# YuliangXiu/ICON

Hardware: NVIDIA H100
Metric: M query-points/sec at 256^3 grid (higher is better)
Workload: dtype f32

## Files before the change

icon_b200/csrc/common.cuh:

```cuda
#pragma once
#include <cuda_runtime.h>
#include <stdint.h>
#include <stdio.h>

#include "../../include/icon_b200.h"

namespace icon {

void set_error(const char *fmt, ...);
void count_launch(int n = 1);

#define ICON_CHECK_ARG(cond, ...)                 \
    do {                                          \
        if (!(cond)) {                            \
            icon::set_error(__VA_ARGS__);         \
            return ICON_EINVAL;                   \
        }                                         \
    } while (0)

#define ICON_CUDA(expr)                                                              \
    do {                                                                             \
        cudaError_t _e = (expr);                                                     \
        if (_e != cudaSuccess) {                                                     \
            icon::set_error("%s:%d %s -> %s", __FILE__, __LINE__, #expr,             \
// ... 57 lines not shown
    template <typename T>
    T *take(size_t n) {
        off = align_up(off, 256);
        T *r = (T *)(base ? base + off : nullptr);
        off += n * sizeof(T);
        return r;
    }
    size_t total() const { return align_up(off, 256); }
};

constexpr int BVH_MAX_LEVELS = 10;
constexpr int RAY_GRID = 256;
constexpr int RAY_LIST_PER_FACE = 64;

constexpr int BRICK_AX = 32;
constexpr int NBRICK = BRICK_AX * BRICK_AX * BRICK_AX;
constexpr int BRICK_MAX_LEAVES = 4096;
constexpr int64_t BRICK_LIST_CAP = 1 << 24;
static inline int64_t brick_list_cap(int F) {
    const int64_t all = (int64_t)NBRICK * ((F + 3) / 4);
    return all < BRICK_LIST_CAP ? all : BRICK_LIST_CAP;
}

struct MeshHeader {
    float y0, z0, inv_cy, inv_cz;
    int ray_overflow;
    int brick_built;
    int brick_overflow;
    int pad;
};

struct MeshView {
    const float4 *tri;
    const float4 *sph;
    const float4 *attr;
    const float4 *rbox;
    float *vnormals;
    unsigned long long *keys;
    int32_t *order;
    float4 *tri_s;
    float4 *sph_s;
    float4 *nodes;
    int32_t *rcount;
    int32_t *roff;
    int32_t *rlist;
    MeshHeader *hdr;
    void *scan_ws;
    float4 *bxyz;
    int32_t *bperm;
    float *brec;
    int32_t *bface;
    float *bub;
    int32_t *boff;
    unsigned short *blist;
    int64_t brick_cap;
    int V, F;
    int nlevels;
    int lvl_cnt[BVH_MAX_LEVELS];
    int lvl_off[BVH_MAX_LEVELS];
};
size_t mesh_ws_bytes(int V, int F);
MeshView mesh_view(const void *ws, int V, int F);
void bricks_forget(const MeshView &m);

void profile_mark(int i, cudaStream_t stream);

size_t scan_ws_bytes(int64_t n);
int scan_exclusive_i32(const int32_t *in, int32_t *out, int64_t n, int64_t *d_total ,
                       void *ws, cudaStream_t stream);

}
```

icon_b200/csrc/mlp.cu:

```cuda
#include "common.cuh"
#include "query_common.cuh"

namespace icon {

constexpr int MP = 64;
constexpr int MT = 256;
constexpr int KC = 16;

constexpr int OFF_W0 = 0;
constexpr int OFF_B0 = OFF_W0 + 16 * 512;
constexpr int OFF_W1 = OFF_B0 + 512;
constexpr int OFF_B1 = OFF_W1 + 512 * 256;
constexpr int OFF_W2 = OFF_B1 + 256;
constexpr int OFF_B2 = OFF_W2 + 272 * 128;
constexpr int OFF_W3 = OFF_B2 + 128;
constexpr int OFF_B3 = OFF_W3 + 144;
static_assert(OFF_B3 + 1 == ICON_MLP_PACKED_FLOATS, "packed layout");

template <int MODE>
__global__ void __launch_bounds__(MT, 2) k_query_mlp(QueryParams q) {
    extern __shared__ __align__(16) float sm[];
    float *x0s = sm;
    float *stage = sm + 16 * MP;
    float *h1s = stage + 10240;
// ... 168 lines not shown
        const float *hb = (st < 16 ? h1s + (size_t)st * KC * MP : x0s) + tx * 4;
#pragma unroll
        for (int k = 0; k < KC; ++k) {
            float4 a0 = *(const float4 *)(wb + k * 128);
            float4 b0 = *(const float4 *)(hb + k * MP), b1 = *(const float4 *)(hb + k * MP + 32);
            float a[4] = {a0.x, a0.y, a0.z, a0.w};
            float b[8] = {b0.x, b0.y, b0.z, b0.w, b1.x, b1.y, b1.z, b1.w};
#pragma unroll
            for (int i = 0; i < 4; ++i)
#pragma unroll
                for (int j = 0; j < 8; ++j) acc2[i][j] = fmaf(a[i], b[j], acc2[i][j]);
        }
        __syncthreads();
    }

    float part[8];
#pragma unroll
    for (int j = 0; j < 8; ++j) part[j] = 0.f;
#pragma unroll
    for (int i = 0; i < 4; ++i) {
        const int ch = ty * 4 + i;
        const float bia = __ldg(W + OFF_B2 + ch), w3 = __ldg(W + OFF_W3 + ch);
#pragma unroll
        for (int j = 0; j < 8; ++j) part[j] = fmaf(w3, lrelu(acc2[i][j] + bia), part[j]);
    }
#pragma unroll
    for (int j = 0; j < 8; ++j) {
        part[j] += __shfl_xor_sync(0xffffffffu, part[j], 8);
        part[j] += __shfl_xor_sync(0xffffffffu, part[j], 16);
    }
    const int lane = tid & 31, wid = tid >> 5;
    if (lane < 8) {
#pragma unroll
        for (int j = 0; j < 4; ++j) {
            red[wid * MP + lane * 4 + j] = part[j];
            red[wid * MP + 32 + lane * 4 + j] = part[4 + j];
        }
    }
    __syncthreads();
    if (tid < MP) {
        const int64_t pi = p0 + tid;
        if (pi < q.N) {
            float s = 0.f;
#pragma unroll
            for (int w = 0; w < 8; ++w) s += red[w * MP + tid];
            for (int j = 0; j < 16; ++j) s = fmaf(__ldg(W + OFF_W3 + 128 + j), x0s[j * MP + tid], s);
            s += __ldg(W + OFF_B3);
            float in_cube = (MODE == 3) ? 1.f : q.xyz4[pi].w;
            q.out[pi] = in_cube * s;
        }
    }
}

__global__ void k_outlier_flag(const float *__restrict__ rec, int64_t N, float clip, int32_t *__restrict__ flag) {
    int64_t i = (int64_t)blockIdx.x * blockDim.x + threadIdx.x;
    if (i < N) flag[i] = fabsf(rec[8 * i]) >= clip ? 1 : 0;
}
__global__ void k_outlier_signs(const float *__restrict__ rec, int64_t N, float clip,
                                const int32_t *__restrict__ krank, int8_t *__restrict__ signs) {
    int64_t i = (int64_t)blockIdx.x * blockDim.x + threadIdx.x;
    if (i < N) {
        float s = rec[8 * i];
        if (fabsf(s) >= clip) signs[krank[i]] = s > 0.f ? 1 : -1;
    }
}

constexpr size_t MLP_SMEM = (16 * MP + 10240 + 256 * MP) * sizeof(float);

template <int MODE>
static int launch_mlp(const QueryParams &q, cudaStream_t stream) {
    static bool attr_set[ICON_MAX_DEVICES] = {};
    if (device_needs_setup(attr_set))
        ICON_CUDA(cudaFuncSetAttribute(k_query_mlp<MODE>, cudaFuncAttributeMaxDynamicSharedMemorySize, (int)MLP_SMEM));
    unsigned nblk = (unsigned)((q.N + MP - 1) / MP);
    k_query_mlp<MODE><<<nblk, MT, MLP_SMEM, stream>>>(q);
    ICON_LAUNCHED();
    return ICON_OK;
}

int launch_mlp_tc(int mode, const QueryParams &q, const void *blob, cudaStream_t stream);
static int g_mlp_impl = 1;

template <int MODE>
static int launch_any(const QueryParams &q, const void *tc, cudaStream_t stream) {
    if (g_mlp_impl == 1) {
        if (!tc) {
            set_error("icon_query / icon_mlp_only: the tensor-core MLP needs the packed tensor-core weight blob (mlp_tc == NULL); "
                      "pass it or select the FP32 kernel with icon_set_mlp_impl(0)");
            return ICON_EINVAL;
        }
        if (q.c0 > 15) {
            set_error("icon_query / icon_mlp_only: the tensor-core MLP takes c0 <= 15 input channels (got %d)", q.c0);
            return ICON_EINVAL;
        }
        return launch_mlp_tc(MODE, q, tc, stream);
    }
    return launch_mlp<MODE>(q, stream);
}

size_t sdf_ws_bytes(int64_t N);
int run_sdf(const float *points, int64_t sc, int64_t sn, int64_t N, const float *h_calib, const MeshView &m,
            float *rec, int32_t *face, void *ws, float4 **xyz4_out, cudaStream_t stream);
int run_points_only(const float *points, int64_t sc, int64_t sn, int64_t N, const float *h_calib,
                    float4 *xyz4, cudaStream_t stream);

struct QueryWs {
    void *sdf_ws;
    float *rec;
    int32_t *krank;
    int8_t *signs;
    int64_t *d_K;
    void *scan_ws;
    float4 *xyz4;
};

static QueryWs carve_query(Carver &c, int64_t N, int prior) {
    QueryWs w{};
    if (prior == ICON_PRIOR_ICON) {
        w.sdf_ws = c.take<char>(sdf_ws_bytes(N));
        w.rec = c.take<float>((size_t)N * 8);
        w.krank = c.take<int32_t>((size_t)N);
        w.signs = c.take<int8_t>((size_t)N);
        w.d_K = c.take<int64_t>(1);
        w.scan_ws = c.take<char>(scan_ws_bytes(N));
    } else {
        w.xyz4 = c.take<float4>((size_t)N);
    }
    return w;
}

}

using namespace icon;

extern "C" size_t icon_query_workspace_bytes(int64_t N, int F, int prior) {
    (void)F;
    Carver c(nullptr);
    carve_query(c, N, prior);
    return c.total();
}

extern "C" int icon_query(int prior, const float *points, int64_t stride_c, int64_t stride_n, int64_t N,
                          const float *h_calib, const float *feat, int C, int H, int W,
                          const float *vol_feat, int VD, const void *mesh_ws, int V, int F,
                          const float *mlp_packed, const void *mlp_tc, int c0, float sdf_clip, float *out,
                          void *ws, size_t ws_bytes, icon_stream_t stream_) {
    cudaStream_t stream = (cudaStream_t)stream_;
    ICON_CHECK_ARG(N >= 0 && N < (int64_t)INT32_MAX, "icon_query: N=%lld out of range", (long long)N);
    if (N == 0) return ICON_OK;
    ICON_CHECK_ARG(points && h_calib && feat && mlp_packed && out && ws, "icon_query: null pointer");
    ICON_CHECK_ARG(((uintptr_t)mlp_tc & 15) == 0, "icon_query: mlp_tc must be 16-byte aligned");
    ICON_CHECK_ARG(c0 >= 1 && c0 <= 16, "icon_query: c0=%d unsupported (1..16)", c0);
    ICON_CHECK_ARG(H >= 2 && W >= 2, "icon_query: feature map %dx%d too small", H, W);
    {
        Carver c(nullptr);
        carve_query(c, N, prior);
        if (ws_bytes < c.total()) {
            set_error("icon_query: workspace %zu < %zu", ws_bytes, c.total());
            return ICON_ENOSPC;
        }
    }
    Carver c(ws);
    QueryWs w = carve_query(c, N, prior);
    QueryParams q{};
    q.feat = feat; q.C = C; q.H = H; q.W = W; q.vol = vol_feat; q.VD = VD;
    q.mlp = mlp_packed; q.c0 = c0; q.clip = sdf_clip; q.out = out; q.N = N;
    if (prior == ICON_PRIOR_ICON) {
        ICON_CHECK_ARG(mesh_ws && V > 0 && F > 0, "icon_query: icon prior needs a prepared body mesh");
        ICON_CHECK_ARG(C % 2 == 0 && C / 2 + 7 == c0, "icon_query: icon prior expects c0 = C/2 + 7 (C=%d c0=%d)", C, c0);
        MeshView m = mesh_view(mesh_ws, V, F);
        float4 *xyz4 = nullptr;
        int rc = run_sdf(points, stride_c, stride_n, N, h_calib, m, w.rec, nullptr, w.sdf_ws, &xyz4, stream);
        if (rc) return rc;
        unsigned nb = (unsigned)((N + 255) / 256);
        k_outlier_flag<<<nb, 256, 0, stream>>>(w.rec, N, sdf_clip, w.krank);
        ICON_LAUNCHED();
        rc = scan_exclusive_i32(w.krank, w.krank, N, w.d_K, w.scan_ws, stream);
        if (rc) return rc;
        k_outlier_signs<<<nb, 256, 0, stream>>>(w.rec, N, sdf_clip, w.krank, w.signs);
        ICON_LAUNCHED();
        q.xyz4 = xyz4; q.rec = w.rec; q.krank = w.krank; q.signs = w.signs; q.d_K = w.d_K;
        profile_mark(3, stream);
        rc = launch_any<0>(q, mlp_tc, stream);
        profile_mark(4, stream);
        return rc;
    }
    profile_mark(0, stream);
    int rc = run_points_only(points, stride_c, stride_n, N, h_calib, w.xyz4, stream);
    if (rc) return rc;
    profile_mark(1, stream); profile_mark(2, stream); profile_mark(3, stream);
    q.xyz4 = w.xyz4;
    if (prior == ICON_PRIOR_PIFU) {
        ICON_CHECK_ARG(C + 1 == c0, "icon_query: pifu prior expects c0 = C + 1 (C=%d c0=%d)", C, c0);
        rc = launch_any<1>(q, mlp_tc, stream);
        profile_mark(4, stream);
        return rc;
    }
    if (prior == ICON_PRIOR_PAMIR) {
        ICON_CHECK_ARG(vol_feat && VD >= 2 && C + 7 == c0, "icon_query: pamir prior expects vol_feat and c0 = C + 7");
        rc = launch_any<2>(q, mlp_tc, stream);
        profile_mark(4, stream);
        return rc;
    }
    set_error("icon_query: unknown prior %d", prior);
    return ICON_EINVAL;
}

extern "C" int icon_set_mlp_impl(int impl) {
    ICON_CHECK_ARG(impl == 0 || impl == 1, "icon_set_mlp_impl: 0 (fp32) or 1 (tensor cores)");
    g_mlp_impl = impl;
    return ICON_OK;
}
extern "C" int icon_get_mlp_impl(void) { return g_mlp_impl; }

extern "C" int icon_mlp_only(const float *feature, int c0, int64_t N, const float *mlp_packed, const void *mlp_tc,
                             float *out, icon_stream_t stream_) {
    cudaStream_t stream = (cudaStream_t)stream_;
    if (N == 0) return ICON_OK;
    ICON_CHECK_ARG(feature && mlp_packed && out && c0 >= 1 && c0 <= 16, "icon_mlp_only: bad argument");
    QueryParams q{};
    q.raw = feature; q.mlp = mlp_packed; q.c0 = c0; q.out = out; q.N = N;
    return launch_any<3>(q, mlp_tc, stream);
}
```

icon_b200/csrc/sdf.cu:

```cuda
#include <float.h>
#include <stdlib.h>

#include <algorithm>
#include <mutex>
#include <type_traits>
#include <unordered_set>

#include "common.cuh"
#include "geom.cuh"

namespace icon {

struct Calib {
    float r[9];
    float t[3];
};

__device__ __forceinline__ V3 load_point(const float *__restrict__ pts, int64_t sc, int64_t sn,
                                         int64_t i, const Calib &cb) {
    float px = pts[i * sn], py = pts[sc + i * sn], pz = pts[2 * sc + i * sn];
    V3 o;
    o.x = fmaf(cb.r[2], pz, fmaf(cb.r[1], py, cb.r[0] * px)) + cb.t[0];
    o.y = fmaf(cb.r[5], pz, fmaf(cb.r[4], py, cb.r[3] * px)) + cb.t[1];
    o.z = fmaf(cb.r[8], pz, fmaf(cb.r[7], py, cb.r[6] * px)) + cb.t[2];
    return o;
}

__device__ __forceinline__ void emit_record(V3 p, int bi, float best, int hits, const MeshView &m,
                                            float *__restrict__ rec, int32_t *__restrict__ face,
                                            int64_t idx) {
    Tri t = load_tri(m.tri + 3 * (size_t)bi);
    V3 n = cross3(t.ab, t.ac);
    float s = n.x * n.x + n.y * n.y + n.z * n.z;
    if (s == 0.f) s = 1e-6f;
    float inv = 1.0f / s;
    V3 w = sub3(p, t.a);
    V3 uw = cross3(t.ab, w), wv = cross3(w, t.ac);
    float b2 = (uw.x * n.x + uw.y * n.y + uw.z * n.z) * inv;
    float b1 = (wv.x * n.x + wv.y * n.y + wv.z * n.z) * inv;
    float b0 = 1.0f - b1 - b2;
    const float4 *at = m.attr + 6 * (size_t)bi;
    float4 a0 = __ldg(at), a1 = __ldg(at + 1), a2 = __ldg(at + 2), a3 = __ldg(at + 3),
           a4 = __ldg(at + 4), a5 = __ldg(at + 5);
    float nx = (a0.x * b0 + a0.w * b1 + a1.z * b2) * -1.f;
    float ny = (a0.y * b0 + a1.x * b1 + a1.w * b2) * 1.f;
    float nz = (a0.z * b0 + a1.y * b1 + a2.x * b2) * -1.f;
    float cx = a2.y * b0 + a3.x * b1 + a3.w * b2;
    float cy = a2.z * b0 + a3.y * b1 + a4.x * b2;
    float cz = a2.w * b0 + a3.z * b1 + a4.y * b2;
    float vv = a4.z * b0 + a4.w * b1 + a5.x * b2;
    float vis = vv >= 0.1f ? 1.f : 0.f;
    float dist = sqrtf(best) / sqrtf(3.0f);
    float sign = 2.0f * ((float)(hits & 1) - 0.5f);
    float sdf = dist * sign;
    float4 *r = (float4 *)(rec + 8 * idx);
    r[0] = make_float4(sdf, cx, cy, cz);
    r[1] = make_float4(nx, ny, nz, vis);
    if (face) face[idx] = bi;
}

constexpr int SW_T = 128;
constexpr int NBIN_AX = 128;
constexpr int NBIN = NBIN_AX * NBIN_AX * NBIN_AX;
__host__ __device__ constexpr int fr_cap(int ppw) { return ppw >= 16 ? 1024 : (ppw >= 4 ? 768 : 384); }

__device__ __forceinline__ float box_dist2(V3 p, float4 lo, float4 hi) {
    float dx = fmaxf(fmaxf(lo.x - p.x, p.x - hi.x), 0.f);
    float dy = fmaxf(fmaxf(lo.y - p.y, p.y - hi.y), 0.f);
    float dz = fmaxf(fmaxf(lo.z - p.z, p.z - hi.z), 0.f);
    return fmaf(dz, dz, fmaf(dy, dy, dx * dx));
}

__device__ __forceinline__ unsigned spread7(unsigned v) {
    v = (v | (v << 16)) & 0x030000FFu;
    v = (v | (v << 8)) & 0x0300F00Fu;
    v = (v | (v << 4)) & 0x030C30C3u;
    v = (v | (v << 2)) & 0x09249249u;
    return v;
}

__device__ __forceinline__ int bin_of(V3 p) {
    const bool inside = p.x >= -1.f && p.x <= 1.f && p.y >= -1.f && p.y <= 1.f && p.z >= -1.f && p.z <= 1.f;
    if (!inside) return NBIN;
    const unsigned bx = min(NBIN_AX - 1, (int)((p.x + 1.f) * (NBIN_AX * 0.5f)));
    const unsigned by = min(NBIN_AX - 1, (int)((p.y + 1.f) * (NBIN_AX * 0.5f)));
    const unsigned bz = min(NBIN_AX - 1, (int)((p.z + 1.f) * (NBIN_AX * 0.5f)));
    return (int)(spread7(bx) | (spread7(by) << 1) | (spread7(bz) << 2));
}

__global__ void k_points_bin(const float *__restrict__ pts, int64_t sc, int64_t sn, int64_t N, Calib cb,
                             float4 *__restrict__ xyz4, int32_t *__restrict__ bid, int32_t *__restrict__ count) {
    const int64_t i = (int64_t)blockIdx.x * blockDim.x + threadIdx.x;
    const bool live = i < N;
    int b = -1;
    if (live) {
        const V3 p = load_point(pts, sc, sn, i, cb);
        const float in_cube = (p.x > -1.f && p.x < 1.f && p.y > -1.f && p.y < 1.f && p.z > -1.f && p.z < 1.f) ? 1.f : 0.f;
        xyz4[i] = make_float4(p.x, p.y, p.z, in_cube);
        b = bin_of(p);
        bid[i] = b;
    }
    const unsigned act = __ballot_sync(0xffffffffu, live);
    if (live) {
        const unsigned peers = __match_any_sync(act, b);
        if ((int)(threadIdx.x & 31) == __ffs(peers) - 1) atomicAdd(&count[b], __popc(peers));
    }
}

__global__ void k_points_scatter(const int32_t *__restrict__ bid, int64_t N, const int32_t *__restrict__ offset,
                                 int32_t *__restrict__ cursor, int32_t *__restrict__ perm) {
    const int64_t i = (int64_t)blockIdx.x * blockDim.x + threadIdx.x;
// ... 17 lines not shown
__device__ __forceinline__ float warp_min(float v) {
    for (int o = 16; o; o >>= 1) v = fminf(v, __shfl_xor_sync(0xffffffffu, v, o));
    return v;
}

#ifdef ICON_SDF_STATS
__device__ unsigned long long g_stats[8];
#define STAT(i, v) do { if (lane == 0) atomicAdd(&g_stats[i], (unsigned long long)(v)); } while (0)
#else
#define STAT(i, v) do { } while (0)
#endif

struct ChunkSmem {
    float4 sph[32];
    float4 tri[32][3];
    int kk[32];
};
template <int FR_CAP>
struct WarpSmem : ChunkSmem {
    unsigned short fr[2][FR_CAP];
};
template <int PPW, bool BRICK>
using SdfSmem = typename std::conditional<BRICK, ChunkSmem, WarpSmem<fr_cap(PPW)>>::type;
template <int PPW, bool BRICK>
constexpr size_t sdf_smem_bytes() { return sizeof(SdfSmem<PPW, BRICK>) * (SW_T / 32); }

constexpr float BRICK_W = 2.0f / BRICK_AX;
constexpr float BRICK_HALF_DIAG = 0.0541266f;

__device__ __forceinline__ void brick_box(int b, float4 &lo, float4 &hi) {
    const int bx = b % BRICK_AX, by = (b / BRICK_AX) % BRICK_AX, bz = b / (BRICK_AX * BRICK_AX);
    lo = make_float4(-1.f + bx * BRICK_W, -1.f + by * BRICK_W, -1.f + bz * BRICK_W, 0.f);
    hi = make_float4(-1.f + (bx + 1) * BRICK_W, -1.f + (by + 1) * BRICK_W, -1.f + (bz + 1) * BRICK_W, 0.f);
}

__device__ __forceinline__ float leaf_key(const MeshView &m, int l, float4 lo, float4 hi) {
    const float4 a = __ldg(m.nodes + 2 * (size_t)l), z = __ldg(m.nodes + 2 * (size_t)l + 1);
    const float gx = fmaxf(fmaxf(a.x - hi.x, lo.x - z.x), 0.f);
    const float gy = fmaxf(fmaxf(a.y - hi.y, lo.y - z.y), 0.f);
    const float gz = fmaxf(fmaxf(a.z - hi.z, lo.z - z.z), 0.f);
    return fmaf(gz, gz, fmaf(gy, gy, gx * gx));
}

__device__ __forceinline__ float box_far2(V3 p, float4 lo, float4 hi) {
    float dx = fmaxf(fabsf(lo.x - p.x), fabsf(hi.x - p.x));
    float dy = fmaxf(fabsf(lo.y - p.y), fabsf(hi.y - p.y));
    float dz = fmaxf(fabsf(lo.z - p.z), fabsf(hi.z - p.z));
    return fmaf(dz, dz, fmaf(dy, dy, dx * dx));
}

template <int PPW, bool BRICK>
__device__ __forceinline__ void sdf_warp(int64_t wid, SdfSmem<PPW, BRICK> &S, const float4 *__restrict__ xyz4,
                                         const int32_t *__restrict__ perm, int64_t N, const MeshView &m,
                                         float *__restrict__ rec, int32_t *__restrict__ face, int order,
                                         int32_t *__restrict__ defer, int32_t *__restrict__ ndefer) {
    constexpr int REP = 32 / PPW;
    constexpr int FR_CAP = fr_cap(PPW);
    const int lane = threadIdx.x & 31;
    const int sub = lane % PPW, rep_id = lane / PPW;
    const int64_t pos0 = wid * PPW;
    const int64_t pos = pos0 + sub;
    if (pos0 >= N) return;
    const bool live = pos < N;
    const int64_t idx = perm[live ? pos : pos0];
    const float4 q = xyz4[idx];
    const V3 p = mk3(q.x, q.y, q.z);
    const V3 c = mk3(0.5f * (warp_min(p.x) + warp_max(p.x)), 0.5f * (warp_min(p.y) + warp_max(p.y)),
                     0.5f * (warp_min(p.z) + warp_max(p.z)));
    const float rw = warp_max(sqrtf(dot3(sub3(p, c), sub3(p, c)))) * 1.00001f + 1e-6f;
    const float4 wlo = make_float4(warp_min(p.x) - 1e-6f, warp_min(p.y) - 1e-6f, warp_min(p.z) - 1e-6f, 0.f);
    const float4 whi = make_float4(warp_max(p.x) + 1e-6f, warp_max(p.y) + 1e-6f, warp_max(p.z) + 1e-6f, 0.f);
    const MeshHeader h = *m.hdr;

    float best = FLT_MAX;
    int bi = 0x7fffffff;
    float ubw2;
    int cur = 0, n = 1;
    bool overflow = false;
    int b = 0;
    float4 blo, bhi;
    if constexpr (BRICK) {
        bool ok = h.brick_built && !h.brick_overflow && c.x >= -1.f && c.x < 1.f && c.y >= -1.f && c.y < 1.f &&
                  c.z >= -1.f && c.z < 1.f;
        if (ok) {
            const int bx = min(BRICK_AX - 1, (int)((c.x + 1.f) * (BRICK_AX * 0.5f)));
            const int by = min(BRICK_AX - 1, (int)((c.y + 1.f) * (BRICK_AX * 0.5f)));
            const int bz = min(BRICK_AX - 1, (int)((c.z + 1.f) * (BRICK_AX * 0.5f)));
            b = (bz * BRICK_AX + by) * BRICK_AX + bx;
            brick_box(b, blo, bhi);
            ok = wlo.x >= blo.x && wlo.y >= blo.y && wlo.z >= blo.z && whi.x <= bhi.x && whi.y <= bhi.y && whi.z <= bhi.z;
        }
        if (!ok) {
            if (lane == 0) defer[atomicAdd(ndefer, 1)] = (int32_t)wid;
            return;
        }
        const int f = __ldg(m.bface + b);
        const Tri tr = load_tri(m.tri + 3 * (size_t)f);
        best = tri_sqdist(p, tr.a, tr.ab, tr.ac);
        bi = f;
        ubw2 = fminf(warp_max(sqrtf(best)), __ldg(m.bub + b));
        STAT(0, 1);
    } else {
        auto try_face = [&](int k) {
            const Tri tr = load_tri(m.tri_s + 3 * (size_t)k);
            const float d = tri_sqdist(p, tr.a, tr.ab, tr.ac);
            const int f = __ldg(m.order + k);
            if (d < best || (d == best && f < bi)) { best = d; bi = f; }
// ... 58 lines not shown
        }
        if (order && !overflow && n > 8) {
            const float ubmin = warp_min(best * rsqrtf(fmaxf(best, 1e-30f))) * 1.00001f + 1e-6f;
            const float t2 = ubmin * ubmin;
            int n1 = 0, n2 = 0;
            for (int base = 0; base < n; base += 32) {
                const int slot = base + lane;
                const bool valid = slot < n;
                int leaf = 0;
                bool near = false;
                if (valid) {
                    leaf = (int)S.fr[cur][slot];
                    const float4 lo = __ldg(m.nodes + 2 * (size_t)leaf), hi = __ldg(m.nodes + 2 * (size_t)leaf + 1);
                    const float gx = fmaxf(fmaxf(lo.x - whi.x, wlo.x - hi.x), 0.f);
                    const float gy = fmaxf(fmaxf(lo.y - whi.y, wlo.y - hi.y), 0.f);
                    const float gz = fmaxf(fmaxf(lo.z - whi.z, wlo.z - hi.z), 0.f);
                    near = fmaf(gz, gz, fmaf(gy, gy, gx * gx)) <= t2;
                }
                const unsigned mn = __ballot_sync(0xffffffffu, valid && near), mf = __ballot_sync(0xffffffffu, valid && !near);
                const unsigned lt = (1u << lane) - 1u;
                if (valid && near) S.fr[cur ^ 1][n1 + __popc(mn & lt)] = (unsigned short)leaf;
                if (valid && !near) S.fr[cur ^ 1][n - 1 - (n2 + __popc(mf & lt))] = (unsigned short)leaf;
                n1 += __popc(mn); n2 += __popc(mf);
            }
            cur ^= 1;
            __syncwarp();
        }
        STAT(0, 1); STAT(1, overflow ? 1 : 0); STAT(2, n);
    }
    {
        float sbA = best * rsqrtf(best) * 1.00001f + 1e-6f;
        float ubA = ubw2 * 1.00001f + 1e-6f;
        auto lane_test = [&](int k, float4 s, const float4 *tr) {
            const float dx = p.x - s.x, dy = p.y - s.y, dz = p.z - s.z;
            const float dd = fmaf(dz, dz, fmaf(dy, dy, dx * dx));
            const float l = sbA + s.w;
            if (dd > l * l) return;
            const float4 r0 = tr[0], r1 = tr[1], r2 = tr[2];
            const V3 ab = mk3(r0.w, r1.x, r1.y), ac = mk3(r1.z, r1.w, r2.x);
            const float S1 = fmaf(dz, ab.z, fmaf(dy, ab.y, dx * ab.x));
            const float T1 = fmaf(dz, ac.z, fmaf(dy, ac.y, dx * ac.x));
            const float M = fmaxf(fmaxf(-(S1 + T1), fmaf(2.f, S1, -T1)), fmaf(2.f, T1, -S1)) * (1.f / 3.f);
            const float g = dd - M - 1e-7f;
            if (g > 0.f && g * g > best * dd * 1.0001f) return;
            const float d = tri_sqdist(p, mk3(r0.x, r0.y, r0.z), ab, ac);
            if (d > best) return;
            const int f = __ldg(m.order + k);
            if (d < best || f < bi) {
                best = d; bi = f;
                sbA = d * rsqrtf(d) * 1.00001f + 1e-6f;
                if (!(d > 0.f)) sbA = 1e-6f;
            }
        };
        auto chunk = [&](int leaf) {
            bool pass = false;
            int k = 0;
            float4 s = make_float4(0.f, 0.f, 0.f, 0.f);
            if (leaf >= 0) {
                k = 4 * leaf + (lane & 3);
                if (k < m.F) {
                    s = __ldg(m.sph_s + k);
                    const float l2 = ubA + s.w;
                    pass = box_dist2(mk3(s.x, s.y, s.z), wlo, whi) <= l2 * l2;
                }
            }
            const unsigned mask = __ballot_sync(0xffffffffu, pass);
            const int cnt = __popc(mask);
            STAT(3, cnt);
            if (pass) {
                const int at = __popc(mask & ((1u << lane) - 1u));
                const float4 *tp = m.tri_s + 3 * (size_t)k;
                S.sph[at] = s;
                S.kk[at] = k;
                S.tri[at][0] = __ldg(tp); S.tri[at][1] = __ldg(tp + 1); S.tri[at][2] = __ldg(tp + 2);
            }
            __syncwarp();
            for (int j = rep_id; j < cnt; j += REP) lane_test(S.kk[j], S.sph[j], &S.tri[j][0]);
            if (REP > 1) {
#pragma unroll
                for (int o = PPW; o < 32; o <<= 1) {
                    const float ob = __shfl_xor_sync(0xffffffffu, best, o);
                    const int oi = __shfl_xor_sync(0xffffffffu, bi, o);
                    if (ob < best || (ob == best && oi < bi)) { best = ob; bi = oi; }
                }
                sbA = best > 0.f ? best * rsqrtf(best) * 1.00001f + 1e-6f : 1e-6f;
            }
            ubA = fminf(ubA, warp_max(sbA));
            __syncwarp();
        };
        if constexpr (BRICK) {
            const int o1 = __ldg(m.boff + b + 1);
            for (int base = __ldg(m.boff + b); base < o1; base += 8) {
                const int slot = base + (lane >> 2);
                const int leaf = slot < o1 ? (int)__ldg(m.blist + slot) : -1;
                float key = 0.f;
                if (lane == 0) key = leaf_key(m, leaf, blo, bhi);
                if (__shfl_sync(0xffffffffu, key, 0) > ubA * ubA) break;
                STAT(2, min(8, o1 - base));
                chunk(leaf);
            }
        } else if (!overflow) {
            for (int base = 0; base < n; base += 8) {
                const int slot = base + (lane >> 2);
                chunk(slot < n ? (int)S.fr[cur][slot] : -1);
            }
        } else {
            for (int k = rep_id; k < m.F; k += REP) {
                lane_test(k, __ldg(m.sph_s + k), m.tri_s + 3 * (size_t)k);
            }
        }
        if (REP > 1) {
#pragma unroll
            for (int o = PPW; o < 32; o <<= 1) {
                const float ob = __shfl_xor_sync(0xffffffffu, best, o);
                const int oi = __shfl_xor_sync(0xffffffffu, bi, o);
                if (ob < best || (ob == best && oi < bi)) { best = ob; bi = oi; }
            }
        }
    }
    int hits = 0;
    if (!h.ray_overflow) {
        const float fy = (p.y - h.y0) * h.inv_cy, fz = (p.z - h.z0) * h.inv_cz;
        if (fy >= 0.f && fy < (float)RAY_GRID && fz >= 0.f && fz < (float)RAY_GRID) {
            const int cc = (int)fz * RAY_GRID + (int)fy;
            const int k0 = __ldg(m.roff + cc), k1 = __ldg(m.roff + cc + 1);
            for (int k = k0 + rep_id; k < k1; k += REP) {
                const int f = __ldg(m.rlist + k);
                if (__ldg(&m.rbox[2 * (size_t)f + 1].x) < p.x - 1e-3f) continue;
                const Tri tr = load_tri(m.tri + 3 * (size_t)f);
                hits += ray_hit_px(p, tr.a, tr.ab, tr.ac);
            }
        }
    } else {
        for (int f = rep_id; f < m.F; f += REP) {
            const Tri tr = load_tri(m.tri + 3 * (size_t)f);
            hits += ray_hit_px(p, tr.a, tr.ab, tr.ac);
        }
    }
    if (REP > 1) {
#pragma unroll
        for (int o = PPW; o < 32; o <<= 1) hits += __shfl_xor_sync(0xffffffffu, hits, o);
    }
    if (live && rep_id == 0) emit_record(p, bi, best, hits, m, rec, face, idx);
}

template <int PPW, bool BRICK>
__global__ void __launch_bounds__(SW_T) k_sdf_warp(const float4 *__restrict__ xyz4, const int32_t *__restrict__ perm,
                                                   int64_t N, MeshView m, float *__restrict__ rec,
                                                   int32_t *__restrict__ face, int order, int32_t *__restrict__ defer,
                                                   int32_t *__restrict__ ndefer) {
    static_assert(!BRICK || PPW == 32, "brick lists serve dense lattices: 32 points per warp");
    extern __shared__ __align__(16) unsigned char smem_raw[];
    SdfSmem<PPW, BRICK> &S = reinterpret_cast<SdfSmem<PPW, BRICK> *>(smem_raw)[threadIdx.x >> 5];
    const bool listed = !BRICK && defer != nullptr;
    const int64_t nw = listed ? (int64_t)*ndefer : (N + PPW - 1) / PPW;
    for (int64_t i = (int64_t)blockIdx.x * (SW_T / 32) + (threadIdx.x >> 5); i < nw; i += (int64_t)gridDim.x * (SW_T / 32))
        sdf_warp<PPW, BRICK>(listed ? (int64_t)defer[i] : i, S, xyz4, perm, N, m, rec, face, order, defer, ndefer);
}

__global__ void k_brick_centres(MeshView m) {
    const int b = blockIdx.x * blockDim.x + threadIdx.x;
    if (b >= NBRICK) return;
    float4 lo, hi;
    brick_box(b, lo, hi);
    m.bxyz[b] = make_float4(0.5f * (lo.x + hi.x), 0.5f * (lo.y + hi.y), 0.5f * (lo.z + hi.z), 0.f);
    m.bperm[b] = b;
}

__global__ void __launch_bounds__(128) k_brick_count(MeshView m) {
    __shared__ int s_cnt;
    const int b = blockIdx.x;
    float4 lo, hi;
    brick_box(b, lo, hi);
    const float4 cc = m.bxyz[b];
    const Tri t = load_tri(m.tri + 3 * (size_t)m.bface[b]);
    const float d = tri_sqdist(mk3(cc.x, cc.y, cc.z), t.a, t.ab, t.ac);
    const float ub = (sqrtf(d) + BRICK_HALF_DIAG) * 1.00001f + 1e-6f, ub2 = ub * ub;
    if (threadIdx.x == 0) s_cnt = 0;
    __syncthreads();
    int cnt = 0;
    for (int l = threadIdx.x; l < m.lvl_cnt[0]; l += blockDim.x) cnt += leaf_key(m, l, lo, hi) <= ub2;
    for (int o = 16; o; o >>= 1) cnt += __shfl_xor_sync(0xffffffffu, cnt, o);
    if ((threadIdx.x & 31) == 0) atomicAdd(&s_cnt, cnt);
    __syncthreads();
    if (threadIdx.x == 0) {
        m.bub[b] = ub;
        m.boff[b] = s_cnt;
        if (s_cnt > BRICK_MAX_LEAVES) m.hdr->brick_overflow = 1;
        if (b == 0) m.boff[NBRICK] = 0;
    }
}

__global__ void __launch_bounds__(128) k_brick_fill(MeshView m, int64_t cap) {
    __shared__ float s_key[BRICK_MAX_LEAVES];
    __shared__ unsigned short s_leaf[BRICK_MAX_LEAVES];
    __shared__ int s_wcnt[4];
    if (m.hdr->brick_overflow || m.boff[NBRICK] > cap) return;
    const int b = blockIdx.x, o0 = m.boff[b], lane = threadIdx.x & 31, wib = threadIdx.x >> 5;
    float4 lo, hi;
    brick_box(b, lo, hi);
    const float ub = m.bub[b], ub2 = ub * ub;
    const int nleaf = m.lvl_cnt[0];
    int n = 0;
    for (int l0 = 0; l0 < nleaf; l0 += 128) {
        const int l = l0 + threadIdx.x;
        float key = 0.f;
        if (l < nleaf) key = leaf_key(m, l, lo, hi);
        const bool in = l < nleaf && key <= ub2;
        const unsigned bal = __ballot_sync(0xffffffffu, in);
        if (lane == 0) s_wcnt[wib] = __popc(bal);
        __syncthreads();
        int at = n + __popc(bal & ((1u << lane) - 1u));
        for (int w = 0; w < wib; ++w) at += s_wcnt[w];
        if (in) { s_key[at] = key; s_leaf[at] = (unsigned short)l; }
        n += s_wcnt[0] + s_wcnt[1] + s_wcnt[2] + s_wcnt[3];
        __syncthreads();
    }
    for (int i = threadIdx.x; i < n; i += blockDim.x) {
        const float k = s_key[i];
        int r = 0;
        for (int j = 0; j < n; ++j) {
            const float kj = s_key[j];
            r += kj < k || (kj == k && j < i);
        }
        m.blist[o0 + r] = s_leaf[i];
    }
}

__global__ void k_brick_done(MeshView m, int64_t cap) {
    if (m.boff[NBRICK] > cap) m.hdr->brick_overflow = 1;
    m.hdr->brick_built = 1;
}

__global__ void __launch_bounds__(256) k_sdf_brute(const float *__restrict__ pts, int64_t sc, int64_t sn,
                                                   int64_t N, Calib cb, MeshView m,
                                                   float *__restrict__ rec, int32_t *__restrict__ face) {
    __shared__ float4 tile[3 * 256];
    int64_t i = (int64_t)blockIdx.x * blockDim.x + threadIdx.x;
    bool live = i < N;
    V3 p = mk3(0.f, 0.f, 0.f);
    if (live) p = load_point(pts, sc, sn, i, cb);
    float best = FLT_MAX;
    int bi = 0, hits = 0;
    for (int f0 = 0; f0 < m.F; f0 += 256) {
        int nf = min(256, m.F - f0);
        __syncthreads();
        for (int k = threadIdx.x; k < 3 * nf; k += 256) tile[k] = m.tri[3 * (size_t)f0 + k];
        __syncthreads();
        if (live) {
            for (int k = 0; k < nf; ++k) {
                float4 r0 = tile[3 * k], r1 = tile[3 * k + 1], r2 = tile[3 * k + 2];
                V3 a = mk3(r0.x, r0.y, r0.z), ab = mk3(r0.w, r1.x, r1.y), ac = mk3(r1.z, r1.w, r2.x);
                float d = tri_sqdist(p, a, ab, ac);
                if (d < best) { best = d; bi = f0 + k; }
                hits += ray_hit_px(p, a, ab, ac);
            }
        }
    }
    if (live) emit_record(p, bi, best, hits, m, rec, face, i);
}

static int64_t g_sdf_ppw32_from = 6000000, g_sdf_ppw8_from = 300000;
static int g_sdf_order = -1;
static int g_sdf_ppw_force = 0;
static int g_sdf_bricks = 1;
static int64_t g_brick_max_entries = 0;

static std::mutex g_brick_mu;
static std::unordered_set<const void *> g_brick_ready;
static int64_t g_brick_builds = 0;

void bricks_forget(const MeshView &m) {
    std::lock_guard<std::mutex> lk(g_brick_mu);
    g_brick_ready.erase(m.hdr);
}

struct SdfWs {
    float4 *xyz4;
    int32_t *bid, *perm, *count, *offset;
    int32_t *defer, *ndefer;
    void *scan_ws;
};
static SdfWs carve_sdf(Carver &c, int64_t N) {
    SdfWs w;
    w.xyz4 = c.take<float4>((size_t)N);
    w.bid = c.take<int32_t>((size_t)N);
    w.perm = c.take<int32_t>((size_t)N);
    w.count = c.take<int32_t>(NBIN + 1);
    w.offset = c.take<int32_t>(NBIN + 1);
    w.defer = c.take<int32_t>((size_t)(N + 31) / 32);
    w.ndefer = c.take<int32_t>(1);
    w.scan_ws = c.take<char>(scan_ws_bytes(NBIN + 1));
    return w;
}

static int build_bricks(const MeshView &m, cudaStream_t stream) {
    const int64_t cap = g_brick_max_entries > 0 ? std::min(g_brick_max_entries, m.brick_cap) : m.brick_cap;
    k_brick_centres<<<NBRICK / 256, 256, 0, stream>>>(m);
    ICON_LAUNCHED();
    k_sdf_warp<1, false><<<NBRICK / (SW_T / 32), SW_T, sdf_smem_bytes<1, false>(), stream>>>(
        m.bxyz, m.bperm, NBRICK, m, m.brec, m.bface, 0, nullptr, nullptr);
    ICON_LAUNCHED();
    k_brick_count<<<NBRICK, 128, 0, stream>>>(m);
    ICON_LAUNCHED();
    int rc = scan_exclusive_i32(m.boff, m.boff, NBRICK + 1, nullptr, m.scan_ws, stream);
    if (rc) return rc;
    k_brick_fill<<<NBRICK, 128, 0, stream>>>(m, cap);
    ICON_LAUNCHED();
    k_brick_done<<<1, 1, 0, stream>>>(m, cap);
    ICON_LAUNCHED();
    return ICON_OK;
}
size_t sdf_ws_bytes(int64_t N) {
    Carver c(nullptr);
    carve_sdf(c, N);
    return c.total();
}

Calib make_calib(const float *h) {
    Calib cb;
    for (int r = 0; r < 3; ++r) {
        for (int k = 0; k < 3; ++k) cb.r[3 * r + k] = h[4 * r + k];
        cb.t[r] = h[4 * r + 3];
    }
    return cb;
}

int run_sdf(const float *points, int64_t sc, int64_t sn, int64_t N, const float *h_calib,
            const MeshView &m, float *rec, int32_t *face, void *ws, float4 **xyz4_out,
            cudaStream_t stream) {
    Carver c(ws);
    SdfWs w = carve_sdf(c, N);
    Calib cb = make_calib(h_calib);
    profile_mark(0, stream);
    ICON_CUDA(cudaMemsetAsync(w.count, 0, sizeof(int32_t) * (NBIN + 1), stream));
    const unsigned nblk = (unsigned)((N + 255) / 256);
    k_points_bin<<<nblk, 256, 0, stream>>>(points, sc, sn, N, cb, w.xyz4, w.bid, w.count);
    ICON_LAUNCHED();
    int rc = scan_exclusive_i32(w.count, w.offset, NBIN + 1, nullptr, w.scan_ws, stream);
    if (rc) return rc;
    ICON_CUDA(cudaMemsetAsync(w.count, 0, sizeof(int32_t) * (NBIN + 1), stream));
    k_points_scatter<<<nblk, 256, 0, stream>>>(w.bid, N, w.offset, w.count, w.perm);
    ICON_LAUNCHED();
    static bool attr_set[ICON_MAX_DEVICES] = {};
    if (device_needs_setup(attr_set)) {
#define ICON_SDF_ATTR(P, B) ICON_CUDA(cudaFuncSetAttribute(k_sdf_warp<P, B>, cudaFuncAttributeMaxDynamicSharedMemorySize, \
                                                           (int)sdf_smem_bytes<P, B>()))
        ICON_SDF_ATTR(32, true); ICON_SDF_ATTR(32, false); ICON_SDF_ATTR(16, false); ICON_SDF_ATTR(8, false);
        ICON_SDF_ATTR(4, false); ICON_SDF_ATTR(2, false); ICON_SDF_ATTR(1, false);
#undef ICON_SDF_ATTR
    }
    profile_mark(1, stream);
    int ppw = N >= g_sdf_ppw32_from ? 32 : (N >= g_sdf_ppw8_from ? 8 : 1);
    if (g_sdf_ppw_force) ppw = g_sdf_ppw_force;
    if (g_sdf_order < 0) {
        const char *e = getenv("ICON_B200_SDF_ORDER");
        g_sdf_order = (e && e[0] == '1') ? 1 : 0;
    }
    const int wpb = SW_T / 32;
    const int64_t nwarps = (N + ppw - 1) / ppw;
    const unsigned nblk_w = (unsigned)((nwarps + wpb - 1) / wpb);
#define ICON_SDF_LAUNCH(P) k_sdf_warp<P, false><<<nblk_w, SW_T, sdf_smem_bytes<P, false>(), stream>>>( \
        w.xyz4, w.perm, N, m, rec, face, g_sdf_order, nullptr, nullptr)
    if (ppw == 32 && g_sdf_bricks) {
        bool build;
        {
            std::lock_guard<std::mutex> lk(g_brick_mu);
            build = g_brick_ready.insert(m.hdr).second;
        }
        if (build) {
            rc = build_bricks(m, stream);
            std::lock_guard<std::mutex> lk(g_brick_mu);
            if (rc) { g_brick_ready.erase(m.hdr); return rc; }
            ++g_brick_builds;
        }
        ICON_CUDA(cudaMemsetAsync(w.ndefer, 0, sizeof(int32_t), stream));
        k_sdf_warp<32, true><<<nblk_w, SW_T, sdf_smem_bytes<32, true>(), stream>>>(
            w.xyz4, w.perm, N, m, rec, face, g_sdf_order, w.defer, w.ndefer);
        ICON_LAUNCHED();
        const unsigned nblk_d = (unsigned)std::min<int64_t>(nblk_w, (int64_t)device_sm_count() * 16);
        k_sdf_warp<32, false><<<nblk_d, SW_T, sdf_smem_bytes<32, false>(), stream>>>(
            w.xyz4, w.perm, N, m, rec, face, g_sdf_order, w.defer, w.ndefer);
    } else {
        switch (ppw) {
            case 32: ICON_SDF_LAUNCH(32); break;
            case 16: ICON_SDF_LAUNCH(16); break;
            case 8: ICON_SDF_LAUNCH(8); break;
            case 4: ICON_SDF_LAUNCH(4); break;
            case 2: ICON_SDF_LAUNCH(2); break;
            default: ICON_SDF_LAUNCH(1); break;
        }
    }
#undef ICON_SDF_LAUNCH
    ICON_LAUNCHED();
    profile_mark(2, stream);
    if (xyz4_out) *xyz4_out = w.xyz4;
    return ICON_OK;
}

__global__ void k_points_only(const float *__restrict__ pts, int64_t sc, int64_t sn, int64_t N, Calib cb,
                              float4 *__restrict__ xyz4) {
    int64_t i = (int64_t)blockIdx.x * blockDim.x + threadIdx.x;
    if (i >= N) return;
    V3 p = load_point(pts, sc, sn, i, cb);
    float in_cube = (p.x > -1.f && p.x < 1.f && p.y > -1.f && p.y < 1.f && p.z > -1.f && p.z < 1.f) ? 1.f : 0.f;
    xyz4[i] = make_float4(p.x, p.y, p.z, in_cube);
}

int run_points_only(const float *points, int64_t sc, int64_t sn, int64_t N, const float *h_calib,
                    float4 *xyz4, cudaStream_t stream) {
    Calib cb = make_calib(h_calib);
    k_points_only<<<(unsigned)((N + 255) / 256), 256, 0, stream>>>(points, sc, sn, N, cb, xyz4);
    ICON_LAUNCHED();
    return ICON_OK;
}

}

using namespace icon;

#ifdef ICON_SDF_STATS
extern "C" int icon_debug_sdf_stats(unsigned long long *out, int reset) {
    cudaMemcpyFromSymbol(out, icon::g_stats, sizeof(unsigned long long) * 8);
    if (reset) { unsigned long long z[8] = {0}; cudaMemcpyToSymbol(icon::g_stats, z, sizeof(z)); }
    return 0;
}
#endif

extern "C" int icon_set_sdf_policy(int force_ppw, int64_t ppw8_from, int64_t ppw32_from) {
    ICON_CHECK_ARG(force_ppw >= 0 && force_ppw <= 32 && (force_ppw & (force_ppw - 1)) == 0, "icon_set_sdf_policy: ppw in {0,1,2,4,8,16,32}");
    icon::g_sdf_ppw_force = force_ppw;
    if (ppw8_from >= 0) icon::g_sdf_ppw8_from = ppw8_from;
    if (ppw32_from >= 0) icon::g_sdf_ppw32_from = ppw32_from;
    return ICON_OK;
}

extern "C" int icon_set_sdf_bricks(int enable, int64_t max_entries) {
    ICON_CHECK_ARG(enable == 0 || enable == 1, "icon_set_sdf_bricks: enable must be 0 or 1");
    icon::g_sdf_bricks = enable;
    icon::g_brick_max_entries = max_entries > 0 ? max_entries : 0;
    return ICON_OK;
}

extern "C" int icon_sdf_brick_info(const void *mesh_ws, int V, int F, int64_t *out) {
    ICON_CHECK_ARG(mesh_ws && out && V > 0 && F > 0, "icon_sdf_brick_info: bad argument");
    MeshView m = mesh_view(mesh_ws, V, F);
    MeshHeader h;
    int32_t total = 0;
    ICON_CUDA(cudaDeviceSynchronize());
    ICON_CUDA(cudaMemcpy(&h, m.hdr, sizeof(h), cudaMemcpyDeviceToHost));
    if (h.brick_built) ICON_CUDA(cudaMemcpy(&total, m.boff + NBRICK, sizeof(total), cudaMemcpyDeviceToHost));
    out[0] = h.brick_built;
    out[1] = h.brick_overflow;
    out[2] = total;
    out[3] = m.brick_cap;
    {
        std::lock_guard<std::mutex> lk(icon::g_brick_mu);
        out[4] = icon::g_brick_builds;
    }
    return ICON_OK;
}

extern "C" int icon_sdf_only(const float *points, int64_t stride_c, int64_t stride_n, int64_t N,
                             const float *h_calib, const void *mesh_ws, int V, int F, float *rec,
                             int32_t *face, void *ws, size_t ws_bytes, icon_stream_t stream_) {
    cudaStream_t stream = (cudaStream_t)stream_;
    ICON_CHECK_ARG(N >= 0 && N < (int64_t)INT32_MAX, "icon_sdf_only: N=%lld out of range", (long long)N);
    if (N == 0) return ICON_OK;
    ICON_CHECK_ARG(points && h_calib && mesh_ws && rec && ws, "icon_sdf_only: null pointer");
    if (ws_bytes < sdf_ws_bytes(N)) {
        set_error("icon_sdf_only: workspace %zu < %zu", ws_bytes, sdf_ws_bytes(N));
        return ICON_ENOSPC;
    }
    MeshView m = mesh_view(mesh_ws, V, F);
    return run_sdf(points, stride_c, stride_n, N, h_calib, m, rec, face, ws, nullptr, stream);
}

extern "C" int icon_sdf_bruteforce(const float *points, int64_t stride_c, int64_t stride_n, int64_t N,
                                   const float *h_calib, const void *mesh_ws, int V, int F, float *rec,
                                   int32_t *face, icon_stream_t stream_) {
    cudaStream_t stream = (cudaStream_t)stream_;
    if (N == 0) return ICON_OK;
    ICON_CHECK_ARG(points && h_calib && mesh_ws && rec, "icon_sdf_bruteforce: null pointer");
    MeshView m = mesh_view(mesh_ws, V, F);
    Calib cb = make_calib(h_calib);
    k_sdf_brute<<<(unsigned)((N + 255) / 256), 256, 0, stream>>>(points, stride_c, stride_n, N, cb, m, rec, face);
    ICON_LAUNCHED();
    return ICON_OK;
}
```

icon_b200/csrc/smpl.cu:

```cuda
#include <float.h>

#include "common.cuh"
#include "geom.cuh"

namespace icon {

static void bvh_levels(int F, int &nlevels, int *cnt, int *off) {
    int n = (F + 3) / 4, l = 0, o = 0;
    while (true) {
        cnt[l] = n; off[l] = o; o += n; ++l;
        if (n == 1 || l == BVH_MAX_LEVELS) break;
        n = (n + 3) / 4;
    }
    nlevels = l;
}

static MeshView carve_mesh(Carver &c, int V, int F) {
    MeshView m{};
    m.V = V; m.F = F;
    bvh_levels(F, m.nlevels, m.lvl_cnt, m.lvl_off);
    const size_t total_nodes = (size_t)m.lvl_off[m.nlevels - 1] + m.lvl_cnt[m.nlevels - 1];
    m.tri = c.take<float4>((size_t)F * 3);
    m.sph = c.take<float4>((size_t)F);
    m.attr = c.take<float4>((size_t)F * 6);
    m.rbox = c.take<float4>((size_t)F * 2);
    m.keys = c.take<unsigned long long>((size_t)F);
    m.order = c.take<int32_t>((size_t)F);
    m.tri_s = c.take<float4>((size_t)F * 3);
    m.sph_s = c.take<float4>((size_t)F);
    m.nodes = c.take<float4>(total_nodes * 2);
    m.rcount = c.take<int32_t>(RAY_GRID * RAY_GRID + 1);
    m.roff = c.take<int32_t>(RAY_GRID * RAY_GRID + 1);
    m.rlist = c.take<int32_t>((size_t)F * RAY_LIST_PER_FACE);
    m.hdr = c.take<MeshHeader>(1);
    m.scan_ws = c.take<char>(scan_ws_bytes(RAY_GRID * RAY_GRID + 1));
    m.bxyz = c.take<float4>(NBRICK);
    m.bperm = c.take<int32_t>(NBRICK);
    m.brec = c.take<float>((size_t)NBRICK * 8);
    m.bface = c.take<int32_t>(NBRICK);
    m.bub = c.take<float>(NBRICK);
    m.boff = c.take<int32_t>(NBRICK + 1);
    m.brick_cap = brick_list_cap(F);
    m.blist = c.take<unsigned short>((size_t)m.brick_cap);
    m.vnormals = c.take<float>((size_t)V * 3);
    return m;
}

size_t mesh_ws_bytes(int V, int F) {
    Carver c(nullptr);
    carve_mesh(c, V, F);
    return c.total();
}

MeshView mesh_view(const void *ws, int V, int F) {
    Carver c((void *)ws);
    return carve_mesh(c, V, F);
}

__global__ void __launch_bounds__(128) k_vertex_normals(const float *__restrict__ verts,
                                                        const int64_t *__restrict__ faces, int V, int F,
                                                        float *__restrict__ out) {
    __shared__ int s_faces[3 * 512];
    const int v = blockIdx.x * blockDim.x + threadIdx.x;
    float sx = 0.f, sy = 0.f, sz = 0.f;
    for (int pass = 0; pass < 3; ++pass) {
        const int corner = (pass == 0) ? 1 : (pass == 1 ? 2 : 0);
        const int c1 = (corner + 1) % 3, c2 = (corner + 2) % 3;
        for (int f0 = 0; f0 < F; f0 += 512) {
            const int nf = min(512, F - f0);
            __syncthreads();
            for (int k = threadIdx.x; k < 3 * nf; k += blockDim.x) s_faces[k] = (int)faces[3 * (size_t)f0 + k];
            __syncthreads();
            if (v < V) {
                for (int k = 0; k < nf; ++k) {
                    if (s_faces[3 * k + corner] != v) continue;
                    const int i1 = s_faces[3 * k + c1], i2 = s_faces[3 * k + c2];
                    V3 p0 = mk3(verts[3 * v], verts[3 * v + 1], verts[3 * v + 2]);
                    V3 p1 = mk3(verts[3 * i1], verts[3 * i1 + 1], verts[3 * i1 + 2]);
                    V3 p2 = mk3(verts[3 * i2], verts[3 * i2 + 1], verts[3 * i2 + 2]);
                    V3 n = cross3(sub3(p1, p0), sub3(p2, p0));
                    sx += n.x; sy += n.y; sz += n.z;
                }
            }
        }
    }
    if (v >= V) return;
    float nrm = sqrtf(sx * sx + sy * sy + sz * sz);
    if (nrm < 1e-6f) nrm = 1e-6f;
    out[3 * v] = sx / nrm;
    out[3 * v + 1] = sy / nrm;
    out[3 * v + 2] = sz / nrm;
}

__device__ __forceinline__ unsigned expand10(unsigned v) {
    v = (v * 0x00010001u) & 0xFF0000FFu;
    v = (v * 0x00000101u) & 0x0F00F00Fu;
// ... 191 lines not shown
```

Baseline: 560.1.

## Pack leaf keys into brick lists, prefetch spheres, fuse outlier flag into SDF

Brick list entries grow from 16-bit leaf ids to 32-bit words whose high half holds the truncated float sort key. The brick loop can then test early termination without calling leaf_key, and it software-pipelines the next entries and face spheres one chunk ahead. The separate outlier-flag kernel is removed, and the SDF emit step now writes the flag directly. This doubles brick list memory traffic and the workspace, and the key comparison uses a truncated float, which is slightly less exact but still conservative.

```diff
diff --git a/icon_b200/csrc/common.cuh b/icon_b200/csrc/common.cuh
--- a/icon_b200/csrc/common.cuh
+++ b/icon_b200/csrc/common.cuh
@@ -133,7 +133,7 @@
     int32_t *bface;
     float *bub;
     int32_t *boff;
-    unsigned short *blist;
+    uint32_t *blist;
     int64_t brick_cap;
     int V, F;
     int nlevels;
diff --git a/icon_b200/csrc/mlp.cu b/icon_b200/csrc/mlp.cu
--- a/icon_b200/csrc/mlp.cu
+++ b/icon_b200/csrc/mlp.cu
@@ -244,10 +244,6 @@
     }
 }
 
-__global__ void k_outlier_flag(const float *__restrict__ rec, int64_t N, float clip, int32_t *__restrict__ flag) {
-    int64_t i = (int64_t)blockIdx.x * blockDim.x + threadIdx.x;
-    if (i < N) flag[i] = fabsf(rec[8 * i]) >= clip ? 1 : 0;
-}
 __global__ void k_outlier_signs(const float *__restrict__ rec, int64_t N, float clip,
                                 const int32_t *__restrict__ krank, int8_t *__restrict__ signs) {
     int64_t i = (int64_t)blockIdx.x * blockDim.x + threadIdx.x;
@@ -292,7 +288,7 @@
 
 size_t sdf_ws_bytes(int64_t N);
 int run_sdf(const float *points, int64_t sc, int64_t sn, int64_t N, const float *h_calib, const MeshView &m,
-            float *rec, int32_t *face, void *ws, float4 **xyz4_out, cudaStream_t stream);
+            float *rec, int32_t *face, int32_t *flag, float clip, void *ws, float4 **xyz4_out, cudaStream_t stream);
 int run_points_only(const float *points, int64_t sc, int64_t sn, int64_t N, const float *h_calib,
                     float4 *xyz4, cudaStream_t stream);
 
@@ -362,11 +358,10 @@
         ICON_CHECK_ARG(C % 2 == 0 && C / 2 + 7 == c0, "icon_query: icon prior expects c0 = C/2 + 7 (C=%d c0=%d)", C, c0);
         MeshView m = mesh_view(mesh_ws, V, F);
         float4 *xyz4 = nullptr;
-        int rc = run_sdf(points, stride_c, stride_n, N, h_calib, m, w.rec, nullptr, w.sdf_ws, &xyz4, stream);
+        int rc = run_sdf(points, stride_c, stride_n, N, h_calib, m, w.rec, nullptr, w.krank, sdf_clip, w.sdf_ws, &xyz4,
+                         stream);
         if (rc) return rc;
         unsigned nb = (unsigned)((N + 255) / 256);
-        k_outlier_flag<<<nb, 256, 0, stream>>>(w.rec, N, sdf_clip, w.krank);
-        ICON_LAUNCHED();
         rc = scan_exclusive_i32(w.krank, w.krank, N, w.d_K, w.scan_ws, stream);
         if (rc) return rc;
         k_outlier_signs<<<nb, 256, 0, stream>>>(w.rec, N, sdf_clip, w.krank, w.signs);
diff --git a/icon_b200/csrc/sdf.cu b/icon_b200/csrc/sdf.cu
--- a/icon_b200/csrc/sdf.cu
+++ b/icon_b200/csrc/sdf.cu
@@ -26,9 +26,15 @@
     return o;
 }
 
+struct SdfOut {
+    float *rec;
+    int32_t *face;
+    int32_t *flag;
+    float clip;
+};
+
 __device__ __forceinline__ void emit_record(V3 p, int bi, float best, int hits, const MeshView &m,
-                                            float *__restrict__ rec, int32_t *__restrict__ face,
-                                            int64_t idx) {
+                                            const SdfOut &out, int64_t idx) {
     Tri t = load_tri(m.tri + 3 * (size_t)bi);
     V3 n = cross3(t.ab, t.ac);
     float s = n.x * n.x + n.y * n.y + n.z * n.z;
@@ -53,10 +59,11 @@
     float dist = sqrtf(best) / sqrtf(3.0f);
     float sign = 2.0f * ((float)(hits & 1) - 0.5f);
     float sdf = dist * sign;
-    float4 *r = (float4 *)(rec + 8 * idx);
+    float4 *r = (float4 *)(out.rec + 8 * idx);
     r[0] = make_float4(sdf, cx, cy, cz);
     r[1] = make_float4(nx, ny, nz, vis);
-    if (face) face[idx] = bi;
+    if (out.face) out.face[idx] = bi;
+    if (out.flag) out.flag[idx] = fabsf(sdf) >= out.clip ? 1 : 0;
 }
 
 constexpr int SW_T = 128;
@@ -180,7 +187,7 @@
 template <int PPW, bool BRICK>
 __device__ __forceinline__ void sdf_warp(int64_t wid, SdfSmem<PPW, BRICK> &S, const float4 *__restrict__ xyz4,
                                          const int32_t *__restrict__ perm, int64_t N, const MeshView &m,
-                                         float *__restrict__ rec, int32_t *__restrict__ face, int order,
+                                         const SdfOut &out, int order,
                                          int32_t *__restrict__ defer, int32_t *__restrict__ ndefer) {
     constexpr int REP = 32 / PPW;
     constexpr int FR_CAP = fr_cap(PPW);
@@ -345,17 +352,16 @@
                 if (!(d > 0.f)) sbA = 1e-6f;
             }
         };
-        auto chunk = [&](int leaf) {
+        auto face_sph = [&](int leaf) {
+            const int k = 4 * leaf + (lane & 3);
+            return leaf >= 0 && k < m.F ? __ldg(m.sph_s + k) : make_float4(0.f, 0.f, 0.f, 0.f);
+        };
+        auto chunk = [&](int leaf, float4 s) {
             bool pass = false;
-            int k = 0;
-            float4 s = make_float4(0.f, 0.f, 0.f, 0.f);
-            if (leaf >= 0) {
-                k = 4 * leaf + (lane & 3);
-                if (k < m.F) {
-                    s = __ldg(m.sph_s + k);
-                    const float l2 = ubA + s.w;
-                    pass = box_dist2(mk3(s.x, s.y, s.z), wlo, whi) <= l2 * l2;
-                }
+            const int k = 4 * leaf + (lane & 3);
+            if (leaf >= 0 && k < m.F) {
+                const float l2 = ubA + s.w;
+                pass = box_dist2(mk3(s.x, s.y, s.z), wlo, whi) <= l2 * l2;
             }
             const unsigned mask = __ballot_sync(0xffffffffu, pass);
             const int cnt = __popc(mask);
@@ -383,19 +389,27 @@
         };
         if constexpr (BRICK) {
             const int o1 = __ldg(m.boff + b + 1);
-            for (int base = __ldg(m.boff + b); base < o1; base += 8) {
+            auto entry = [&](int base) {
                 const int slot = base + (lane >> 2);
-                const int leaf = slot < o1 ? (int)__ldg(m.blist + slot) : -1;
-                float key = 0.f;
-                if (lane == 0) key = leaf_key(m, leaf, blo, bhi);
-                if (__shfl_sync(0xffffffffu, key, 0) > ubA * ubA) break;
+                return slot < o1 ? __ldg(m.blist + slot) : 0xffffffffu;
+            };
+            auto leaf_of = [](unsigned e) { return e == 0xffffffffu ? -1 : (int)(e & 0xffffu); };
+            int base = __ldg(m.boff + b);
+            unsigned e = entry(base), en = entry(base + 8);
+            float4 s = face_sph(leaf_of(e));
+            for (; base < o1; base += 8) {
+                if (__uint_as_float(__shfl_sync(0xffffffffu, e, 0) & 0xffff0000u) > ubA * ubA) break;
                 STAT(2, min(8, o1 - base));
-                chunk(leaf);
+                const float4 sn = face_sph(leaf_of(en));
+                const unsigned enn = entry(base + 16);
+                chunk(leaf_of(e), s);
+                e = en; en = enn; s = sn;
             }
         } else if (!overflow) {
             for (int base = 0; base < n; base += 8) {
                 const int slot = base + (lane >> 2);
-                chunk(slot < n ? (int)S.fr[cur][slot] : -1);
+                const int leaf = slot < n ? (int)S.fr[cur][slot] : -1;
+                chunk(leaf, face_sph(leaf));
             }
         } else {
             for (int k = rep_id; k < m.F; k += REP) {
@@ -434,21 +448,20 @@
 #pragma unroll
         for (int o = PPW; o < 32; o <<= 1) hits += __shfl_xor_sync(0xffffffffu, hits, o);
     }
-    if (live && rep_id == 0) emit_record(p, bi, best, hits, m, rec, face, idx);
+    if (live && rep_id == 0) emit_record(p, bi, best, hits, m, out, idx);
 }
 
 template <int PPW, bool BRICK>
 __global__ void __launch_bounds__(SW_T) k_sdf_warp(const float4 *__restrict__ xyz4, const int32_t *__restrict__ perm,
-                                                   int64_t N, MeshView m, float *__restrict__ rec,
-                                                   int32_t *__restrict__ face, int order, int32_t *__restrict__ defer,
-                                                   int32_t *__restrict__ ndefer) {
+                                                   int64_t N, MeshView m, SdfOut out, int order,
+                                                   int32_t *__restrict__ defer, int32_t *__restrict__ ndefer) {
     static_assert(!BRICK || PPW == 32, "brick lists serve dense lattices: 32 points per warp");
     extern __shared__ __align__(16) unsigned char smem_raw[];
     SdfSmem<PPW, BRICK> &S = reinterpret_cast<SdfSmem<PPW, BRICK> *>(smem_raw)[threadIdx.x >> 5];
     const bool listed = !BRICK && defer != nullptr;
     const int64_t nw = listed ? (int64_t)*ndefer : (N + PPW - 1) / PPW;
     for (int64_t i = (int64_t)blockIdx.x * (SW_T / 32) + (threadIdx.x >> 5); i < nw; i += (int64_t)gridDim.x * (SW_T / 32))
-        sdf_warp<PPW, BRICK>(listed ? (int64_t)defer[i] : i, S, xyz4, perm, N, m, rec, face, order, defer, ndefer);
+        sdf_warp<PPW, BRICK>(listed ? (int64_t)defer[i] : i, S, xyz4, perm, N, m, out, order, defer, ndefer);
 }
 
 __global__ void k_brick_centres(MeshView m) {
@@ -516,7 +529,7 @@
             const float kj = s_key[j];
             r += kj < k || (kj == k && j < i);
         }
-        m.blist[o0 + r] = s_leaf[i];
+        m.blist[o0 + r] = (__float_as_uint(k) & 0xffff0000u) | s_leaf[i];
     }
 }
 
@@ -550,7 +563,7 @@
             }
         }
     }
-    if (live) emit_record(p, bi, best, hits, m, rec, face, i);
+    if (live) emit_record(p, bi, best, hits, m, SdfOut{rec, face, nullptr, 0.f}, i);
 }
 
 static int64_t g_sdf_ppw32_from = 6000000, g_sdf_ppw8_from = 300000;
@@ -592,7 +605,7 @@
     k_brick_centres<<<NBRICK / 256, 256, 0, stream>>>(m);
     ICON_LAUNCHED();
     k_sdf_warp<1, false><<<NBRICK / (SW_T / 32), SW_T, sdf_smem_bytes<1, false>(), stream>>>(
-        m.bxyz, m.bperm, NBRICK, m, m.brec, m.bface, 0, nullptr, nullptr);
+        m.bxyz, m.bperm, NBRICK, m, SdfOut{m.brec, m.bface, nullptr, 0.f}, 0, nullptr, nullptr);
     ICON_LAUNCHED();
     k_brick_count<<<NBRICK, 128, 0, stream>>>(m);
     ICON_LAUNCHED();
@@ -620,10 +633,11 @@
 }
 
 int run_sdf(const float *points, int64_t sc, int64_t sn, int64_t N, const float *h_calib,
-            const MeshView &m, float *rec, int32_t *face, void *ws, float4 **xyz4_out,
+            const MeshView &m, float *rec, int32_t *face, int32_t *flag, float clip, void *ws, float4 **xyz4_out,
             cudaStream_t stream) {
     Carver c(ws);
     SdfWs w = carve_sdf(c, N);
+    const SdfOut out{rec, face, flag, clip};
     Calib cb = make_calib(h_calib);
     profile_mark(0, stream);
     ICON_CUDA(cudaMemsetAsync(w.count, 0, sizeof(int32_t) * (NBIN + 1), stream));
@@ -654,7 +668,7 @@
     const int64_t nwarps = (N + ppw - 1) / ppw;
     const unsigned nblk_w = (unsigned)((nwarps + wpb - 1) / wpb);
 #define ICON_SDF_LAUNCH(P) k_sdf_warp<P, false><<<nblk_w, SW_T, sdf_smem_bytes<P, false>(), stream>>>( \
-        w.xyz4, w.perm, N, m, rec, face, g_sdf_order, nullptr, nullptr)
+        w.xyz4, w.perm, N, m, out, g_sdf_order, nullptr, nullptr)
     if (ppw == 32 && g_sdf_bricks) {
         bool build;
         {
@@ -669,11 +683,11 @@
         }
         ICON_CUDA(cudaMemsetAsync(w.ndefer, 0, sizeof(int32_t), stream));
         k_sdf_warp<32, true><<<nblk_w, SW_T, sdf_smem_bytes<32, true>(), stream>>>(
-            w.xyz4, w.perm, N, m, rec, face, g_sdf_order, w.defer, w.ndefer);
+            w.xyz4, w.perm, N, m, out, g_sdf_order, w.defer, w.ndefer);
         ICON_LAUNCHED();
         const unsigned nblk_d = (unsigned)std::min<int64_t>(nblk_w, (int64_t)device_sm_count() * 16);
         k_sdf_warp<32, false><<<nblk_d, SW_T, sdf_smem_bytes<32, false>(), stream>>>(
-            w.xyz4, w.perm, N, m, rec, face, g_sdf_order, w.defer, w.ndefer);
+            w.xyz4, w.perm, N, m, out, g_sdf_order, w.defer, w.ndefer);
     } else {
         switch (ppw) {
             case 32: ICON_SDF_LAUNCH(32); break;
@@ -766,7 +780,7 @@
         return ICON_ENOSPC;
     }
     MeshView m = mesh_view(mesh_ws, V, F);
-    return run_sdf(points, stride_c, stride_n, N, h_calib, m, rec, face, ws, nullptr, stream);
+    return run_sdf(points, stride_c, stride_n, N, h_calib, m, rec, face, nullptr, 0.f, ws, nullptr, stream);
 }
 
 extern "C" int icon_sdf_bruteforce(const float *points, int64_t stride_c, int64_t stride_n, int64_t N,
diff --git a/icon_b200/csrc/smpl.cu b/icon_b200/csrc/smpl.cu
--- a/icon_b200/csrc/smpl.cu
+++ b/icon_b200/csrc/smpl.cu
@@ -41,7 +41,7 @@
     m.bub = c.take<float>(NBRICK);
     m.boff = c.take<int32_t>(NBRICK + 1);
     m.brick_cap = brick_list_cap(F);
-    m.blist = c.take<unsigned short>((size_t)m.brick_cap);
+    m.blist = c.take<uint32_t>((size_t)m.brick_cap);
     m.vnormals = c.take<float>((size_t)V * 3);
     return m;
 }
```

After: 565.3, median of 6. No clear change (+0.9%).
